# quentinll/pertrenderer

Measured on NVIDIA B200. Metric: perturbed shader fwd+bwd pixel·face·samples/sec, higher is better.
Workload: dtype f32

## Files before the change

pertrenderer_b200/csrc/cabi.cu:

```cuda
#include <math.h>

#include "kernels.h"

using namespace pert;

static thread_local const char* g_last_cuda = "none";

static int cuda_fail(int e) {
    g_last_cuda = cudaGetErrorName((cudaError_t)e);
    return PERT_E_CUDA;
}
static int cuda_rc(int e) { return e == 0 ? PERT_OK : cuda_fail(e); }

extern "C" int pert_version(void) { return PERT_ABI_VERSION; }

extern "C" uint32_t pert_shade_fused_flags(void) {
    return PERT_F_NO_SKIP | PERT_F_SKIP_DEAD_NOISE | PERT_F_PER_SAMPLE_NOISE | PERT_F_CAUCHY | PERT_F_NO_VR | PERT_F_PHILOX7;
}

extern "C" const char* pert_last_cuda_error(void) { return g_last_cuda; }

extern "C" const char* pert_strerror(int code) {
    switch (code) {
        case PERT_OK: return "ok";
// ... 120 lines not shown
static int sparse_cap(int K, int tp) {
    int cap = tp * K / 5;
    cap = (cap + 7) & ~7;
    if (cap < 32) cap = 32;
    if (cap > tp * K) cap = (tp * K + 1) & ~1;
    return cap;
}

static bool sparse_first_ok(const pert_problem* pb, const void* worklist, bool all_phases) {
    if (!worklist || !all_phases || pb->noise_rast || pb->noise_agg) return false;
    if (pb->flags & (PERT_F_NO_SKIP | PERT_F_PER_SAMPLE_NOISE | PERT_F_CAUCHY | PERT_F_NO_VR)) return false;
    return true;
}

static bool cauchy_flags_bad(uint32_t f) {
    return (f & PERT_F_CAUCHY) &&
           (f & (PERT_F_PHILOX7 | PERT_F_NO_VR | PERT_F_SKIP_DEAD_NOISE | PERT_F_UNIFORM | PERT_F_GUMBEL));
}

static bool no_vr_flags_bad(uint32_t f) {
    return (f & PERT_F_NO_VR) && (f & (PERT_F_PHILOX7 | PERT_F_SKIP_DEAD_NOISE | PERT_F_UNIFORM | PERT_F_GUMBEL));
}

extern "C" int64_t pert_num_tiles(const pert_problem* pb) {
    if (!pb || pb->K <= 0) return 0;
    const int64_t P = pb->N * pb->H * pb->W;
    const int a = dense_tp(pb->K, P), b = sparse_tp(pb->K, P);
    const int tp = a < b ? a : b;
    return (P + tp - 1) / tp;
}

extern "C" int pert_winner_bytes(int32_t K) { return (K + 1 <= 256) ? 1 : 2; }

extern "C" int64_t pert_blob_bytes(const pert_problem* pb) {
    if (!pb || pb->K <= 0) return 0;
    const int64_t P = pb->N * pb->H * pb->W;
    const int tp = sparse_tp(pb->K, P);
    return ((P + tp - 1) / tp) * (int64_t)blob_words(tp, sparse_cap(pb->K, tp)) * 4;
}

static bool aligned16(const void* p) { return ((uintptr_t)p & 15) == 0; }

static int fwd_launch_records(FwdArgs& a, FwdArgs& fb, bool sparse) {
    const int64_t P = a.pb.N * a.pb.H * a.pb.W;
    if (sparse) {
        SmemLayout t;
        const int tp2 = sparse_tp(a.pb.K, P) / 2;
        fwd_smem_layout(tp2, tp2 * a.pb.K, t);
        if ((size_t)t.bytes * (FBT / 32) > 200 * 1024) sparse = false;
    }
    a.L = make_launch(&a.pb, sparse ? sparse_tp(a.pb.K, P) : dense_tp(a.pb.K, P));
    a.L.vec_ok = a.L.vec_ok && aligned16(a.pb.pix_to_face);
    if (sparse) a.L.cap = sparse_cap(a.pb.K, a.L.tp);
    fwd_smem_layout(a.L.tp, a.L.cap, a.L.sm);
    a.L.warp_smem = a.L.sm.bytes;
    if ((size_t)a.L.warp_smem > 200 * 1024) return PERT_E_UNSUPPORTED;
    if (a.L.ntiles > 0x7fffffff) return PERT_E_UNSUPPORTED;
    if (!sparse) return 0;
    fb = a;
    fb.blob = nullptr;
    fb.L = make_launch(&a.pb, a.L.tp / 2);
    fb.L.vec_ok = fb.L.vec_ok && aligned16(a.pb.pix_to_face);
    fb.L.warp_smem_rast = fwd_smem_layout(fb.L.tp, fb.L.cap, fb.L.sm);
    fb.L.warp_smem = fb.L.sm.bytes;
    return 1;
}

extern "C" int pert_shade_fwd(const pert_problem* pb_in, float* image, uint16_t* counts, float* rsum, void* winners,
                              uint16_t* pixstate, int32_t* hist, int32_t* worklist, void* tile_blob, void* stream) {
    int rc = check_problem(pb_in);
    if (rc) return rc;
    FwdArgs a;
    a.pb = *pb_in;
    if (!(a.pb.flags & (PERT_PH_RAST | PERT_PH_AGG | PERT_PH_BLEND))) a.pb.flags |= PERT_PH_RAST | PERT_PH_AGG | PERT_PH_BLEND;
    const uint32_t f = a.pb.flags;
    if (!counts) return PERT_E_NULL;
    if ((f & PERT_PH_RAST) && !rsum) return PERT_E_NULL;
    if ((f & PERT_PH_AGG) && (!winners || !pixstate)) return PERT_E_NULL;
    if ((f & PERT_PH_BLEND) && (!image || (!a.pb.colors && !a.pb.face_colors))) return PERT_E_NULL;
    if (((f & PERT_PH_AGG) != 0) != ((f & PERT_PH_BLEND) != 0) && !hist) return PERT_E_NULL;
    if (((uintptr_t)image & 15) || ((uintptr_t)counts & 1) || ((uintptr_t)rsum & 3) || ((uintptr_t)hist & 3) ||
        ((uintptr_t)a.pb.colors & 3) || ((uintptr_t)pixstate & 1) || ((uintptr_t)winners & 3))
        return PERT_E_ALIGN;
    if ((uintptr_t)worklist & 15) return PERT_E_ALIGN;
    const uint32_t all = PERT_PH_RAST | PERT_PH_AGG | PERT_PH_BLEND;
    if ((f & PERT_F_PHILOX7) && ((f & all) != all || hist || a.pb.noise_rast || a.pb.noise_agg)) return PERT_E_UNSUPPORTED;
    if (cauchy_flags_bad(f) || no_vr_flags_bad(f)) return PERT_E_UNSUPPORTED;
    a.image = image;
    a.counts = counts;
    a.rsum = rsum;
    a.winners = winners;
    a.pixstate = pixstate;
    a.hist = hist;
    a.worklist = worklist;
    a.blob = nullptr;
    FwdArgs fb;
    rc = fwd_launch_records(a, fb, sparse_first_ok(&a.pb, worklist, (f & all) == all && !hist));
    if (rc < 0) return rc;
    const bool sparse = rc == 1;
    if ((uintptr_t)tile_blob & 15) return PERT_E_ALIGN;
    a.blob = sparse ? (int32_t*)tile_blob : nullptr;
    cudaStream_t st = (cudaStream_t)stream;
    if (!sparse) return cuda_rc(launch_shade_fwd(a, nullptr, st));
    cudaError_t e = cudaMemsetAsync(worklist, 0, 16, st);
    if (e != cudaSuccess) return cuda_fail((int)e);
    return cuda_rc(launch_shade_fwd(a, &fb, st));
}

extern "C" int pert_shade_render(const pert_problem* pb_in, float* image, uint16_t* counts_ws, int32_t* worklist,
                                 void* stream) {
    int rc = check_problem(pb_in);
    if (rc) return rc;
    FwdArgs a = {};
    a.pb = *pb_in;
    const uint32_t f = a.pb.flags;
    if (f & (PERT_PH_RAST | PERT_PH_AGG | PERT_PH_BLEND | PERT_PH_BWD_SAMPLE | PERT_PH_BWD_FINISH)) return PERT_E_UNSUPPORTED;
    if (a.pb.s_rast_begin != 0 || a.pb.s_rast_end != a.pb.S_rast || a.pb.s_agg_begin != 0 || a.pb.s_agg_end != a.pb.S_agg)
        return PERT_E_UNSUPPORTED;
    if (!image || (!a.pb.colors && !a.pb.face_colors)) return PERT_E_NULL;
    if (((uintptr_t)image & 15) || ((uintptr_t)counts_ws & 1) || ((uintptr_t)a.pb.colors & 3) || ((uintptr_t)worklist & 15))
        return PERT_E_ALIGN;
    if ((f & PERT_F_PHILOX7) && (a.pb.noise_rast || a.pb.noise_agg)) return PERT_E_UNSUPPORTED;
    if (cauchy_flags_bad(f) || no_vr_flags_bad(f)) return PERT_E_UNSUPPORTED;
    if (f & PERT_F_NO_VR) a.pb.flags |= PERT_F_PER_SAMPLE_NOISE;
    const bool sparse_ok = sparse_first_ok(&a.pb, worklist, true);
    if (sparse_ok && !counts_ws) return PERT_E_NULL;
    a.image = image;
    a.counts = counts_ws;
    a.worklist = worklist;
    FwdArgs fb;
    rc = fwd_launch_records(a, fb, sparse_ok);
    if (rc < 0) return rc;
    cudaStream_t st = (cudaStream_t)stream;
    if (rc == 0) return cuda_rc(launch_shade_render(a, nullptr, st));
// ... 32 lines not shown
        const Launch t = make_launch(&a.pb, tp2);
        SmemLayout sl;
        bwd_smem_layout(tp2, a.pb.K, t.cap, t.sc, t.nchunks, t.win_bytes, false, true, sl);
        if ((size_t)sl.bytes * (FBT / 32) > 200 * 1024) sparse = false;
    }
    const bool ptr_ok = aligned16(a.pb.pix_to_face) && aligned16(grad_dists) && aligned16(grad_zbuf) &&
                        (a.pb.face_colors || aligned16(grad_colors));
    a.L = make_launch(&a.pb, sparse ? sparse_tp(a.pb.K, a.pb.N * a.pb.H * a.pb.W) : dense_tp(a.pb.K, a.pb.N * a.pb.H * a.pb.W));
    a.L.vec_ok = a.L.vec_ok && ptr_ok;
    if (sparse) a.L.cap = sparse_cap(a.pb.K, a.L.tp);
    if (a.L.win_bytes == 2 && ((uintptr_t)winners & 1)) return PERT_E_ALIGN;
    bwd_smem_layout(a.L.tp, a.pb.K, a.L.cap, a.L.sc, a.L.nchunks, a.L.win_bytes, sparse, a.L.lean, a.L.sm);
    a.L.warp_smem = a.L.sm.bytes;
    if ((size_t)a.L.warp_smem > 200 * 1024) return PERT_E_UNSUPPORTED;
    if (a.L.ntiles > 0x7fffffff) return PERT_E_UNSUPPORTED;
    a.grad_image = grad_image;
    a.counts = counts;
    a.rsum = rsum;
    a.winners = winners;
    a.pixstate = pixstate;
    a.grad_dists = grad_dists;
    a.grad_zbuf = grad_zbuf;
    a.grad_colors = grad_colors;
    a.partials = scalar_partials;
    a.acc = acc;
    a.pixstat = pixstat;
    a.hist = hist;
    a.worklist = worklist;
    if ((uintptr_t)tile_blob & 15) return PERT_E_ALIGN;
    a.blob = sparse ? (const int32_t*)tile_blob : nullptr;
    cudaStream_t st = (cudaStream_t)stream;
    if (!sparse) return cuda_rc(launch_shade_bwd(a, nullptr, grad_scalars, st));
    BwdArgs fb = a;
    fb.blob = nullptr;
    fb.L = make_launch(&a.pb, a.L.tp / 2);
    fb.L.vec_ok = fb.L.vec_ok && ptr_ok;
    fb.L.lean = true;
    bwd_smem_layout(fb.L.tp, a.pb.K, fb.L.cap, fb.L.sc, fb.L.nchunks, fb.L.win_bytes, false, fb.L.lean, fb.L.sm);
    fb.L.warp_smem = fb.L.sm.bytes;
    cudaError_t e = cudaMemsetAsync(worklist, 0, 16, st);
    if (e != cudaSuccess) return cuda_fail((int)e);
    return cuda_rc(launch_shade_bwd(a, &fb, grad_scalars, st));
}

static int soft_launch_record(pert_problem& pb, Launch& L, bool bwd, bool ptr_ok) {
    pb.S_rast = pb.S_agg = 4;
    pb.s_rast_begin = pb.s_agg_begin = 0;
    pb.s_rast_end = pb.s_agg_end = 4;
    pb.noise_rast = pb.noise_agg = nullptr;
    pb.face_colors = nullptr;
    int rc = check_problem(&pb);
    if (rc) return rc;
    if (!pb.colors) return PERT_E_NULL;
    L = make_launch(&pb, pick_tp(pb.K));
    L.vec_ok = L.vec_ok && ptr_ok;
    soft_smem_layout(L.tp, pb.K, bwd, L.sm);
    L.warp_smem = L.sm.bytes;
    if ((size_t)L.warp_smem > 200 * 1024) return PERT_E_UNSUPPORTED;
    return PERT_OK;
}

extern "C" int pert_soft_shade_fwd(const pert_problem* pb_in, float* image, void* stream) {
    if (!pb_in || !image) return PERT_E_NULL;
    if ((uintptr_t)image & 15) return PERT_E_ALIGN;
    pert_problem pb = *pb_in;
    Launch L;
    if (int rc = soft_launch_record(pb, L, false, aligned16(pb.pix_to_face))) return rc;
// ... 171 lines not shown
```

pertrenderer_b200/csrc/common.cuh:

```cuda
#pragma once
#include <cuda_runtime.h>
#include <math_constants.h>
#include <stdint.h>

#include "../../include/pertshade.h"

namespace pert {

constexpr int NT = 128;
constexpr int NW = NT / 32;
constexpr int FNT = 32;
constexpr int FBT = 64;
constexpr unsigned FULL = 0xffffffffu;

__device__ __forceinline__ float warp_sum(float v) {
#pragma unroll
    for (int o = 16; o > 0; o >>= 1) v += __shfl_xor_sync(FULL, v, o);
    return v;
}
__device__ __forceinline__ int warp_sum_i(int v) {
#pragma unroll
    for (int o = 16; o > 0; o >>= 1) v += __shfl_xor_sync(FULL, v, o);
    return v;
}
// ... 201 lines not shown

__device__ __forceinline__ int best_lane_shift(int n, int nq, int kmax) {
    int best_k = 0, best_c = 0x7fffffff;
#pragma unroll 1
    for (int k = 0; k <= kmax; ++k) {
        const int passes = ((n << k) + 31) >> 5;
        const int per_lane = (nq + (1 << k) - 1) >> k;
        const int c = passes * (per_lane * 100 + 24 + 6 * k);
        if (c < best_c) {
            best_c = c;
            best_k = k;
        }
    }
    return best_k;
}

__device__ __forceinline__ int batch_of(int64_t pix0, int p, int64_t HW) {
    const unsigned hw = (unsigned)HW;
    const unsigned b0 = (unsigned)pix0 / hw;
    unsigned r = (unsigned)pix0 - b0 * hw + (unsigned)p;
    unsigned b = b0;
    while (r >= hw) {
        r -= hw;
        b++;
    }
    return (int)b;
}

__host__ __device__ __forceinline__ int blob_words(int tp, int cap) { return ((2 + 7 * tp + 2 * cap) + 3) & ~3; }
__host__ __device__ __forceinline__ int blob_pix_off(int tp) { return 2 + tp; }
__host__ __device__ __forceinline__ int blob_vlist_off(int tp) { return 2 + 7 * tp; }
__host__ __device__ __forceinline__ int blob_cnt_off(int tp, int cap) { return 2 + 7 * tp + cap / 2; }
__host__ __device__ __forceinline__ int blob_zeta_off(int tp, int cap) { return 2 + 7 * tp + cap; }

__device__ __forceinline__ int entry_pixel(int e, float invK) { return __float2int_rz(((float)e + 0.5f) * invK); }

}
```

pertrenderer_b200/csrc/shade_bwd.cu:

```cuda
#include <climits>
#include "kernels.h"
#include "tile.cuh"

namespace pert {

constexpr int kNab = 8;

void bwd_smem_layout(int tp, int K, int cap, int sc, int nchunks, int win_bytes, bool compact, bool lean, SmemLayout& L) {
    const size_t ns = compact ? (size_t)cap + 2 * tp : (size_t)tp * (K + 1);
    Carver cv(L);
    cv.take(cap, 2);
    cv.take(ns > (size_t)cap ? ns : (size_t)cap, 4);
    cv.take(lean && ns > (size_t)cap ? ns : (size_t)cap, 2);
    cv.take(ns, 4);
    cv.take(ns, 4);
    cv.take(nchunks > 1 ? ns : 0, 4);
    cv.take(lean ? 0 : ns, 2);
    cv.take((size_t)(tp < kNab ? tp : kNab) * sc, 4);
    cv.take(tp + 1, 4);
    cv.take(tp, 4);
    cv.take(tp, 4);
    cv.take(compact ? tp : 0, 4);
    cv.take(compact ? tp : 0, 4);
    cv.take(tp, 1);
// ... 36 lines not shown
    float* gsel = cv.take<float>();
    float* accs = zs;
    float* t2s_own = cv.take<float>();
    float* t2s = a.L.nchunks > 1 ? t2s_own : gsel;
    uint16_t* pairs_own = cv.take<uint16_t>();
    const bool lean = a.L.lean;
    uint16_t* pairs = lean ? cnt : pairs_own;
    float* cs = cv.take<float>();
    int* vstart = cv.take<int>();
    int* pa0 = cv.take<int>();
    float* pg0 = cv.take<float>();
    int* psb = cv.take<int>();
    int* pnv = cv.take<int>();
    uint8_t* apx = cv.take<uint8_t>();
    const bool early_w = a.L.nchunks == 1 && ((sa_loc * wb) & 15) == 0 && do_sample && (((uintptr_t)a.winners) & 15) == 0;
    unsigned char* wst = cv.take<unsigned char>();
    if (early_w) {
        const unsigned char* src = reinterpret_cast<const unsigned char*>(a.winners) + pix0 * sa_loc * wb;
        const int nbytes = npx * sa_loc * wb;
#pragma unroll 1
        for (int o = lane * 16; o < nbytes; o += 32 * 16) cp_async16(wst + o, src + o);
    }

    float4 Gi = make_float4(0.f, 0.f, 0.f, 0.f);
    float zn = 1.0f, zf = 100.0f;
    int pstate = K;
    if (pvalid) {
        Gi = __ldg(reinterpret_cast<const float4*>(a.grad_image) + gp);
        const int b = pb.depth_len > 1 ? batch_of(pix0, p, a.L.HW) : 0;
        zn = __ldg(pb.znear + b);
        zf = __ldg(pb.zfar + b);
        pstate = a.pixstate[gp];
    }
    const int32_t* const bl = BLOB ? a.blob + tile * (int64_t)blob_words(tp, cap) : nullptr;
    const int nv = BLOB ? __ldg(bl) : scan_valid(pb.pix_to_face + g0, E, a.L.vec_ok, vlist, cap);
    const bool overflow = COMPACT && (BLOB ? nv < 0 : nv > cap);
    if (!overflow) {
        if (do_finish) {
            zero_fill(a.grad_dists + g0, E, a.L.vec_ok);
            zero_fill(a.grad_zbuf + g0, E, a.L.vec_ok);
            if (a.grad_colors && !FACE) zero_fill(a.grad_colors + g0 * 3, E * 3, a.L.vec_ok);
        } else {
            zero_fill(a.acc + pix0 * K1, npx * K1, false);
            if (lane < npx) {
                a.pixstat[(pix0 + lane) * 2] = 0.f;
                a.pixstat[(pix0 + lane) * 2 + 1] = 0.f;
            }
        }
    }
    if (overflow) {
        if (lane == 0) a.worklist[4 + atomicAdd(a.worklist, 1)] = (int32_t)tile;
    } else if (nv > 0 || WOVR) {
        const float gal = a.L.gal;
        PixPrep pi;
        if constexpr (BLOB) {
            const float* const colors_t = pb.colors + g0 * 3;
            const float* const rsum_t = a.rsum + g0;
            for (int i = lane; i <= tp; i += 32) vstart[i] = __ldg(bl + 1 + i);
            uint32_t* const vl32 = reinterpret_cast<uint32_t*>(vlist);
            uint32_t* const cn32 = reinterpret_cast<uint32_t*>(cnt);
            const int nw = (nv + 1) >> 1;
#pragma unroll 1
            for (int i = lane; i < nw; i += 32) {
                const uint32_t v2 = (uint32_t)__ldg(bl + blob_vlist_off(tp) + i);
                vl32[i] = v2;
                cn32[i] = (uint32_t)__ldg(bl + blob_cnt_off(tp, cap) + i);
                const int e0 = v2 & 0xffff, e1 = v2 >> 16;
                if (!FACE) prefetch_l1(colors_t + e0 * 3);
                prefetch_l1(rsum_t + e0);
                if (2 * i + 1 < nv) {
                    if (!FACE) prefetch_l1(colors_t + e1 * 3);
                    prefetch_l1(rsum_t + e1);
                }
            }
#pragma unroll 1
            for (int i = lane; i < nv; i += 32) zs[i] = __int_as_float(__ldg(bl + blob_zeta_off(tp, cap) + i));
            if (pvalid) {
                const int32_t* const bp = bl + blob_pix_off(tp) + 6 * p;
                pi.zmax = __int_as_float(__ldg(bp));
                pi.zimax = __int_as_float(__ldg(bp + 1));
                pi.prod_nz = __int_as_float(__ldg(bp + 2));
                pi.zeta_max = __int_as_float(__ldg(bp + 3));
                const int w4 = __ldg(bp + 4), w5 = __ldg(bp + 5);
                pi.argzi = w4 & 0xffff;
                pi.a0 = w4 >> 16;
                pi.nzero = w5 & 0xffff;
                pi.kpad = w5 >> 16;
            } else {
                pi.zmax = pb.eps;
                pi.zimax = 0.f;
                pi.prod_nz = 1.f;
                pi.zeta_max = 0.f;
                pi.argzi = pi.a0 = pi.nzero = pi.kpad = 0;
            }
            pi.zbg = __fadd_rn(pb.eps, -pi.zmax);
            __syncwarp();
        } else {
            __syncwarp();
            pixel_ranges(vlist, nv, K, tp, vstart);
            {
                const float* const zbuf_t = pb.zbuf + g0;
                const uint16_t* const counts_t = a.counts + g0;
                const float* const colors_t = pb.colors + g0 * 3;
                const float* const rsum_t = a.rsum + g0;
#pragma unroll 1
                for (int n = lane; n < nv; n += 32) {
                    const int e = vlist[n];
                    zs[n] = __ldg(zbuf_t + e);
                    cnt[n] = counts_t[e];
// ... 358 lines not shown
                            float* gc = gfc + 3 * (int)__ldg(p2f_p + k);
                            atomicAdd(gc, w * Gi.x);
                            atomicAdd(gc + 1, w * Gi.y);
                            atomicAdd(gc + 2, w * Gi.z);
                        } else {
                            float* gc = gc_t + e * 3;
                            gc[0] = w * Gi.x;
                            gc[1] = w * Gi.y;
                            gc[2] = w * Gi.z;
                        }
                    }
                }
            }
        }
    }

    if (do_finish) {
        p_sigma = warp_sum(p_sigma);
        p_gamma = warp_sum(p_gamma);
        p_q = warp_sum(p_q);
        if (lane == 0) reinterpret_cast<float4*>(a.partials)[prow] = make_float4(p_sigma, p_gamma, p_q, 0.f);
    }
}

constexpr int BWD_MAIN_CTAS = 28;
template <class NoiseA, int GT, bool PHASED, bool FACE, bool COMPACT, bool BLOB, int SCORE = 0, bool WOVR = false>
__global__ void __launch_bounds__(FNT, BWD_MAIN_CTAS) shade_bwd_kernel(const BwdArgs a, const NoiseA noise_a) {
    extern __shared__ __align__(16) unsigned char smem_raw[];
    NoiseA na = noise_a;
    if (a.pb.seed_device) na.mix(__ldg(a.pb.seed_device + 1));
    shade_bwd_tile<NoiseA, GT, PHASED, FACE, COMPACT, BLOB, SCORE, WOVR>(a, na, blockIdx.x, blockIdx.x, smem_raw, threadIdx.x);
}

template <class NoiseA, int GT, bool FACE>
__global__ void __launch_bounds__(FBT, 12) shade_bwd_fallback_kernel(const BwdArgs a, const NoiseA noise_a, int64_t prow0) {
    extern __shared__ __align__(16) unsigned char smem_all[];
    unsigned char* smem_raw = smem_all + (threadIdx.x >> 5) * a.L.warp_smem;
    const int n = 2 * a.worklist[0];
    NoiseA na = noise_a;
    if (a.pb.seed_device) na.mix(__ldg(a.pb.seed_device + 1));
#pragma unroll 1
    for (;;) {
        int i = 0;
        if ((threadIdx.x & 31) == 0) i = n > 0 ? atomicAdd(a.worklist + 1, 1) : 0;
        i = __shfl_sync(FULL, i, 0);
        if (i >= n) break;
        const int64_t tile = (int64_t)a.worklist[4 + (i >> 1)] * 2 + (i & 1);
        if (tile < a.L.ntiles) {
            shade_bwd_tile<NoiseA, GT, false, FACE, false, false>(a, na, tile, prow0 + i, smem_raw, threadIdx.x & 31);
        } else if ((threadIdx.x & 31) == 0) {
            reinterpret_cast<float4*>(a.partials)[prow0 + i] = make_float4(0.f, 0.f, 0.f, 0.f);
        }
        __syncwarp();
    }
}

__global__ void __launch_bounds__(1024) finalize_scalars_kernel(const float* partials, int64_t n, const int32_t* worklist,
                                                                float gamma, float alpha, float* out) {
    __shared__ double red[3][32];
    if (worklist) n += 2 * (int64_t)worklist[0];
    double s0 = 0, s1 = 0, s2 = 0;
    const float4* const rows = reinterpret_cast<const float4*>(partials);
    int64_t t = threadIdx.x;
    for (; t + 7 * 1024 < n; t += 8 * 1024) {
        float4 v[8];
#pragma unroll
        for (int u = 0; u < 8; ++u) v[u] = __ldg(rows + t + u * 1024);
#pragma unroll
        for (int u = 0; u < 8; ++u) {
            s0 += v[u].x;
            s1 += v[u].y;
            s2 += v[u].z;
        }
    }
    for (; t < n; t += 1024) {
        const float4 v = __ldg(rows + t);
        s0 += v.x;
        s1 += v.y;
        s2 += v.z;
    }
#pragma unroll
    for (int o = 16; o > 0; o >>= 1) {
// ... 19 lines not shown
        out[2] = (float)(-q * (double)gamma / ((double)alpha * (double)alpha));
    }
}

template <class K>
static int set_smem(K kern, size_t smem) {
    if (smem > 48 * 1024) return (int)cudaFuncSetAttribute(kern, cudaFuncAttributeMaxDynamicSharedMemorySize, (int)smem);
    return 0;
}

template <class NA, int GT, bool PHASED, bool FACE, bool COMPACT, bool BLOB = false, int SCORE = 0, bool WOVR = false>
static int launch_bwd_f(const BwdArgs& a, const NA& na, cudaStream_t st) {
    const size_t smem = (size_t)a.L.warp_smem;
    if (int rc = set_smem(shade_bwd_kernel<NA, GT, PHASED, FACE, COMPACT, BLOB, SCORE, WOVR>, smem)) return rc;
    shade_bwd_kernel<NA, GT, PHASED, FACE, COMPACT, BLOB, SCORE, WOVR><<<(unsigned)a.L.ntiles, FNT, smem, st>>>(a, na);
    return (int)cudaGetLastError();
}
template <class NA, int GT, bool PHASED, int SCORE = 0, bool WOVR = false>
static int launch_bwd_t(const BwdArgs& a, const NA& na, cudaStream_t st) {
    return a.pb.face_colors ? launch_bwd_f<NA, GT, PHASED, true, false, false, SCORE, WOVR>(a, na, st)
                            : launch_bwd_f<NA, GT, PHASED, false, false, false, SCORE, WOVR>(a, na, st);
}
template <class PN, int GT>
static int launch_bwd_c(const BwdArgs& a, const PN& na, cudaStream_t st) {
    if (a.blob) {
        if constexpr (GT == 2 || GT == 4) {
            return a.pb.face_colors ? launch_bwd_f<PN, GT, false, true, true, true>(a, na, st)
                                    : launch_bwd_f<PN, GT, false, false, true, true>(a, na, st);
        }
    }
    return a.pb.face_colors ? launch_bwd_f<PN, GT, false, true, true>(a, na, st)
                            : launch_bwd_f<PN, GT, false, false, true>(a, na, st);
}
template <class PN, int GT, bool FACE>
static int launch_bwd_fb(const BwdArgs& a, const PN& na, int64_t prow0, cudaStream_t st) {
    const size_t smem = (size_t)a.L.warp_smem * (FBT / 32);
    if (int rc = set_smem(shade_bwd_fallback_kernel<PN, GT, FACE>, smem)) return rc;
    shade_bwd_fallback_kernel<PN, GT, FACE><<<resident_grid(shade_bwd_fallback_kernel<PN, GT, FACE>, FBT, smem), FBT, smem, st>>>(a, na, prow0);
    return (int)cudaGetLastError();
}

template <class PN>
static int launch_bwd_production(const BwdArgs& a, const BwdArgs* fb, cudaStream_t st) {
    const PN pa(a.pb.seed_agg, 1, a.pb.pixel_offset);
    int rc;
    if (fb) {
        switch (a.L.G) {
            case 1: rc = launch_bwd_c<PN, 1>(a, pa, st); break;
            case 2: rc = launch_bwd_c<PN, 2>(a, pa, st); break;
            case 4: rc = launch_bwd_c<PN, 4>(a, pa, st); break;
            default: rc = launch_bwd_c<PN, 8>(a, pa, st); break;
        }
        if (rc) return rc;
        const bool face = a.pb.face_colors != nullptr;
        switch (fb->L.G) {
            case 2: return face ? launch_bwd_fb<PN, 2, true>(*fb, pa, a.L.ntiles, st) : launch_bwd_fb<PN, 2, false>(*fb, pa, a.L.ntiles, st);
            case 4: return face ? launch_bwd_fb<PN, 4, true>(*fb, pa, a.L.ntiles, st) : launch_bwd_fb<PN, 4, false>(*fb, pa, a.L.ntiles, st);
            case 8: return face ? launch_bwd_fb<PN, 8, true>(*fb, pa, a.L.ntiles, st) : launch_bwd_fb<PN, 8, false>(*fb, pa, a.L.ntiles, st);
            default: return face ? launch_bwd_fb<PN, 16, true>(*fb, pa, a.L.ntiles, st) : launch_bwd_fb<PN, 16, false>(*fb, pa, a.L.ntiles, st);
        }
    }
    switch (a.L.G) {
        case 1: return launch_bwd_t<PN, 1, false>(a, pa, st);
        case 2: return launch_bwd_t<PN, 2, false>(a, pa, st);
        case 4: return launch_bwd_t<PN, 4, false>(a, pa, st);
        default: return launch_bwd_t<PN, 8, false>(a, pa, st);
    }
}

int launch_shade_bwd(const BwdArgs& a, const BwdArgs* fb, float* grad_scalars, cudaStream_t st) {
    int rc;
    const uint32_t both = PERT_PH_BWD_SAMPLE | PERT_PH_BWD_FINISH;
// ... 40 lines not shown
```

pertrenderer_b200/csrc/shade_fwd.cu:

```cuda
#include "kernels.h"
#include "tile.cuh"

namespace pert {

int fwd_smem_layout(int tp, int cap, SmemLayout& L) {
    Carver cv(L);
    cv.take(cap, 2);
    cv.take(cap + tp, 4);
    cv.take(cap, 2);
    cv.take(cap + tp, 4);
    cv.take(cap + tp, 2);
    cv.take(64, 2);
    const int rast_bytes = L.bytes;
    cv.take(cap, 4);
    cv.take(tp + 1, 4);
    cv.take(tp, 4);
    cv.take(tp, 2);
    return rast_bytes;
}

constexpr int kDeferMin = 48;
constexpr int kCmpMin = 12;

template <class NoiseR, class NoiseA, int GT, bool PHASED, bool DEFER = false, int CPH = 0x70, int SCORE = 0,
          bool WOVR = false, bool RENDER = false>
__device__ __forceinline__ void shade_fwd_tile(const FwdArgs& a, const NoiseR& noise_r, const NoiseA& noise_a,
                                               const int64_t tile, unsigned char* smem_raw, const int lane) {
    const pert_problem& pb = a.pb;
    const int G = GT ? GT : a.L.G;
    const int gshift = GT ? (GT == 16 ? 4 : GT == 8 ? 3 : GT == 4 ? 2 : GT == 2 ? 1 : 0) : a.L.gshift;
    const int K = pb.K, K1 = K + 1, tp = 32 >> gshift;
    const int64_t pix0 = tile * tp;
    const int npx = (int)min((int64_t)tp, a.L.P - pix0);
    const int E = npx * K;
    const int64_t g0 = pix0 * K;
    const uint32_t flags = pb.flags;
    const bool do_rast = PHASED ? (flags & PERT_PH_RAST) != 0 : (CPH & PERT_PH_RAST) != 0,
               do_agg = PHASED ? (flags & PERT_PH_AGG) != 0 : (CPH & PERT_PH_AGG) != 0,
               do_blend = PHASED ? (flags & PERT_PH_BLEND) != 0 : (CPH & PERT_PH_BLEND) != 0;
    int32_t* const ghist = PHASED ? a.hist : nullptr;
    const float* const zbuf_t = pb.zbuf + g0;
    const float* const dists_t = pb.dists + g0;
    uint16_t* const counts_t = a.counts + g0;
    float* const rsum_t = a.rsum + g0;
    const bool no_skip = flags & PERT_F_NO_SKIP;
    const int p = lane >> gshift, lig = lane & (G - 1);
    const bool pvalid = p < npx;
    const int64_t gp = pix0 + p;
    const unsigned lt = (1u << lane) - 1u;

    Taker cv(smem_raw, a.L.sm);
    uint16_t* vlist = cv.take<uint16_t>();
    float* xs = cv.take<float>();
    uint16_t* cnt = cv.take<uint16_t>();
    float* rs = cv.take<float>();
    uint16_t* rlist = cv.take<uint16_t>();
    uint16_t* ring = cv.take<uint16_t>();
    float* zs = cv.take<float>();
    int* vstart = cv.take<int>();
    int* pinfo = cv.take<int>();
    uint16_t* plist = cv.take<uint16_t>();
    const int cap = a.L.cap;
    float* lz = xs;
    int* hl = reinterpret_cast<int*>(rs);
    uint16_t* lj = rlist;

    const int nv = scan_valid(pb.pix_to_face + g0, E, a.L.vec_ok, vlist, cap);
    const int sa_loc = a.L.sa_loc;
    if (nv > cap) {
        if (lane == 0) {
            a.worklist[4 + atomicAdd(a.worklist, 1)] = (int32_t)tile;
            if (a.blob) a.blob[tile * (int64_t)blob_words(tp, cap)] = -1;
        }
        return;
    }
    if (nv == 0) {
        if (do_agg && ghist) {
#pragma unroll 1
            for (int i = lane; i < npx * K1; i += 32) ghist[pix0 * K1 + i] = ((i % K1) == K) ? sa_loc : 0;
        }
        if (!RENDER && do_agg && lane < npx) a.pixstate[pix0 + lane] = (uint16_t)K;
        if (!PHASED && !RENDER && a.blob && lane == 0) a.blob[tile * (int64_t)blob_words(tp, a.L.cap)] = 0;
        if (do_blend && lane < npx)
            reinterpret_cast<float4*>(a.image)[pix0 + lane] =
                make_float4(pb.background[0], pb.background[1], pb.background[2], 0.0f);
        return;
    }
    __syncwarp();
    if (do_agg || do_blend) pixel_ranges(vlist, nv, K, tp, vstart);

    const int sr_loc = pb.s_rast_end - pb.s_rast_begin;
    const float thr = (NoiseR::kBounded && !no_skip) ? pb.sigma * kNoiseAbsMax * 1.0001f : CUDART_INF_F;
    const bool compound = !WOVR && NoiseR::kBounded && !no_skip && !(flags & PERT_F_PER_SAMPLE_NOISE);
    const float x_cmp = compound ? a.L.t_compound * pb.sigma : CUDART_INF_F;
    uint16_t* const blist = rlist + cap - 1;
    int nlist = 0, nblist = 0;
#pragma unroll 1
    for (int n0 = 0; n0 < nv; n0 += 32) {
        const int n = n0 + lane;
        bool need = false, cmp = false;
        if (n < nv) {
            const int e = vlist[n];
            if (do_agg || do_blend) {
                zs[n] = __ldg(zbuf_t + e);
                if (!pb.face_colors) prefetch_l1(pb.colors + (g0 + e) * 3);
            }
            if (do_rast) {
                const float x = -__ldg(dists_t + e);
                xs[n] = x;
                need = WOVR ? x >= -thr : fabsf(x) <= thr;
                cmp = need && fabsf(x) >= x_cmp;
                if (!need) {
                    cnt[n] = (x >= 0.0f) ? (uint16_t)sr_loc : (uint16_t)0;
                    if constexpr (!RENDER) rs[n] = 0.0f;
                }
            } else {
                cnt[n] = counts_t[e];
            }
        }
        if (do_rast) {
            if constexpr (DEFER) {
                const unsigned b = __ballot_sync(FULL, need);
                if (need) rlist[nlist + __popc(b & lt)] = (uint16_t)n;
                nlist += __popc(b);
                nblist += __popc(__ballot_sync(FULL, cmp));
            } else {
                const unsigned b = __ballot_sync(FULL, need && !cmp), bc = __ballot_sync(FULL, cmp);
                if (need && !cmp) rlist[nlist + __popc(b & lt)] = (uint16_t)n;
                if (cmp) blist[-(nblist + __popc(bc & lt))] = (uint16_t)n;
                nlist += __popc(b);
                nblist += __popc(bc);
            }
        }
    }
    __syncwarp();
    if (do_rast) {
        if constexpr (DEFER) {
            if (nblist >= kDeferMin) {
                if (lane == 0) {
                    a.worklist[4 + atomicAdd(a.worklist, 1)] = (int32_t)tile;
                    if (a.blob) a.blob[tile * (int64_t)blob_words(tp, cap)] = -1;
                }
                return;
            }
        }
        if (!DEFER && nblist > 0 && nblist < kCmpMin) {
            const int moved = lane < nblist ? blist[-lane] : 0;
            __syncwarp();
            if (lane < nblist) rlist[nlist + lane] = (uint16_t)moved;
            nlist += nblist;
            nblist = 0;
            __syncwarp();
        }
        if constexpr (NoiseR::kBounded && !DEFER && !WOVR) {
            if (nblist > 0) {
                const CompoundCtx<NoiseR> cc{noise_r, vlist, xs, cnt, rs, K, a.L.invK, pix0, a.L.inv_sigma, sr_loc,
                                             0x40000000u + 2u * (uint32_t)(pb.s_rast_begin >> 2)};
                if constexpr (RENDER)
                    rast_compound_count_list(cc, blist, nblist, a.L.t_bucket[0] * pb.sigma, a.L.t_bucket[1] * pb.sigma, ring);
                else
                    rast_compound_list(cc, blist, nblist, a.L.t_bucket[0] * pb.sigma, a.L.t_bucket[1] * pb.sigma, ring);
            }
        }
        rast_sample_list<NoiseR, SCORE, WOVR, RENDER>(noise_r, rlist, nlist, vlist, xs, cnt, rs, K, a.L.invK, pix0, pb.sigma, a.L.inv_sigma, pb.s_rast_begin,
                         pb.s_rast_end, !no_skip, a.L.lpe_r);
        __syncwarp();
        if (!RENDER || !do_agg) {
#pragma unroll 1
            for (int n = lane; n < nv; n += 32) {
                const int e = vlist[n];
                counts_t[e] = cnt[n];
                if constexpr (!RENDER) rsum_t[e] = rs[n];
            }
        }
// ... 100 lines not shown
                        }
                    }
                    int wj[4];
#pragma unroll
                    for (int t = 0; t < 4; ++t) {
                        wj[t] = lj[plb + bi[t]];
                        const int s = q * 4 + t;
                        if (s >= pb.s_agg_begin && s < pb.s_agg_end && bi[t] != pa0) atomicAdd(&hl[plb + bi[t]], 1);
                    }
                    if constexpr (RENDER) continue;
                    const int s0 = q * 4 - pb.s_agg_begin;
                    if (pack && q * 4 + 3 < pb.s_agg_end) {
                        reinterpret_cast<uint32_t*>(a.winners)[(pgp * sa_loc + s0) >> 2] =
                            (uint32_t)wj[0] | ((uint32_t)wj[1] << 8) | ((uint32_t)wj[2] << 16) | ((uint32_t)wj[3] << 24);
                    } else {
#pragma unroll
                        for (int t = 0; t < 4; ++t)
                            if (q * 4 + t < pb.s_agg_end) store_winner(a.winners, a.L.win_bytes, pgp * sa_loc + s0 + t, wj[t]);
                    }
                }
            }
        }
        __syncwarp();
        int others = 0;
#pragma unroll 1
        for (int l = lig; l < nlive; l += G)
            if (l != a0l) others += hl[lb + l];
        others = group_sum_i(others, G);
        active = others > 0;
        if (pvalid && lig == 0) {
            hl[lb + a0l] = sa_loc - others;
            if constexpr (!RENDER) a.pixstate[gp] = (uint16_t)(pi.a0 | (active ? 0x8000 : 0));
        }
        if (!PHASED && !RENDER && a.blob) {
            int32_t* const bl = a.blob + tile * (int64_t)blob_words(tp, cap);
            if (lane == 0) bl[0] = nv;
            for (int i = lane; i <= tp; i += 32) bl[1 + i] = i <= npx ? vstart[i] : nv;
            if (pvalid && lig == 0) {
                int32_t* const bp = bl + blob_pix_off(tp) + 6 * p;
                bp[0] = __float_as_int(pi.zmax);
                bp[1] = __float_as_int(pi.zimax);
                bp[2] = __float_as_int(pi.prod_nz);
                bp[3] = __float_as_int(pi.zeta_max);
                bp[4] = pi.argzi | (pi.a0 << 16);
                bp[5] = pi.nzero | (pi.kpad << 16);
            }
            const uint32_t* const vl32 = reinterpret_cast<const uint32_t*>(vlist);
            const uint32_t* const cn32 = reinterpret_cast<const uint32_t*>(cnt);
            const int nw = (nv + 1) >> 1;
#pragma unroll 1
            for (int i = lane; i < nw; i += 32) {
                bl[blob_vlist_off(tp) + i] = (int32_t)vl32[i];
                bl[blob_cnt_off(tp, cap) + i] = (int32_t)cn32[i];
            }
#pragma unroll 1
            for (int i = lane; i < nv; i += 32) bl[blob_zeta_off(tp, cap) + i] = __float_as_int(zs[i]);
        }
        __syncwarp();
        if (ghist) {
#pragma unroll 1
            for (int i = lane; i < npx * K1; i += 32) ghist[pix0 * K1 + i] = 0;
            __syncwarp();
#pragma unroll 1
            for (int l = lig; l < nlive; l += G) ghist[gp * K1 + lj[lb + l]] = hl[lb + l];
        }
    }
    if (!do_blend) return;

    float r = 0.f, g = 0.f, bl = 0.f;
    const float fS = (float)pb.S_agg;
    const float* const colors_p = pb.colors + gp * K * 3;
    const float* const fcol = pb.face_colors;
    const int64_t* const p2f_p = pb.pix_to_face + gp * K;
    if (do_agg) {
#pragma unroll 1
        for (int l = lig; l < nlive; l += G) {
            const int hcount = hl[lb + l];
            if (hcount > 0) {
                const float w = (float)hcount / fS;
                const int j = lj[lb + l];
                if (j < K) {
                    const float* c = fcol ? fcol + 3 * (int)__ldg(p2f_p + j) : colors_p + j * 3;
                    r += w * __ldg(c);
                    g += w * __ldg(c + 1);
                    bl += w * __ldg(c + 2);
                } else {
                    r += w * pb.background[0];
                    g += w * pb.background[1];
                    bl += w * pb.background[2];
// ... 13 lines not shown
                    r += w * __ldg(c);
                    g += w * __ldg(c + 1);
                    bl += w * __ldg(c + 2);
                } else {
                    r += w * pb.background[0];
                    g += w * pb.background[1];
                    bl += w * pb.background[2];
                }
            }
        }
    }
    r = group_sum(r, G);
    g = group_sum(g, G);
    bl = group_sum(bl, G);
    if (pvalid && lig == 0) reinterpret_cast<float4*>(a.image)[gp] = make_float4(r, g, bl, px_alpha);
}

constexpr int fwd_min_ctas(int score, bool wovr, bool render) { return (score || wovr) ? 24 : render ? 28 : 32; }

template <class NoiseR, class NoiseA, int GT, bool PHASED, bool DEFER, int SCORE, bool WOVR, bool RENDER>
__global__ void __launch_bounds__(FNT, fwd_min_ctas(SCORE, WOVR, RENDER))
    shade_fwd_kernel(const FwdArgs a, const NoiseR noise_r, const NoiseA noise_a) {
    extern __shared__ __align__(16) unsigned char smem_raw[];
    NoiseR nr = noise_r;
    NoiseA na = noise_a;
    if (a.pb.seed_device) {
        nr.mix(__ldg(a.pb.seed_device));
        na.mix(__ldg(a.pb.seed_device + 1));
    }
    shade_fwd_tile<NoiseR, NoiseA, GT, PHASED, DEFER, 0x70, SCORE, WOVR, RENDER>(a, nr, na, blockIdx.x, smem_raw, threadIdx.x);
}

constexpr int FB_MIN_CTAS = 12;
template <class PN, int GT, int CPH, bool RENDER>
__global__ void __launch_bounds__(FBT, FB_MIN_CTAS) shade_fwd_fallback_kernel(const FwdArgs a, const PN noise_r, const PN noise_a) {
    extern __shared__ __align__(16) unsigned char smem_all[];
    unsigned char* smem_raw = smem_all + (threadIdx.x >> 5) * (CPH == (int)PERT_PH_RAST ? a.L.warp_smem_rast : a.L.warp_smem);
    const int n = 2 * a.worklist[0];
    PN nr = noise_r;
    PN na = noise_a;
    if (a.pb.seed_device) {
        nr.mix(__ldg(a.pb.seed_device));
        na.mix(__ldg(a.pb.seed_device + 1));
    }
#pragma unroll 1
    for (;;) {
        int i = 0;
        if ((threadIdx.x & 31) == 0) i = n > 0 ? atomicAdd(a.worklist + ((CPH & PERT_PH_RAST) ? 1 : 2), 1) : 0;
        i = __shfl_sync(FULL, i, 0);
        if (i >= n) break;
        const int64_t tile = (int64_t)a.worklist[4 + (i >> 1)] * 2 + (i & 1);
        if (tile < a.L.ntiles)
            shade_fwd_tile<PN, PN, GT, false, false, CPH, 0, false, RENDER>(a, nr, na, tile, smem_raw, threadIdx.x & 31);
        __syncwarp();
    }
}

template <class NR, class NA, int GT, bool PHASED, bool DEFER, int SCORE, bool WOVR, bool RENDER>
static int launch_t(const FwdArgs& a, const NR& nr, const NA& na, cudaStream_t st) {
    const size_t smem = (size_t)a.L.warp_smem;
    if (smem > 48 * 1024) {
        cudaError_t e = cudaFuncSetAttribute(shade_fwd_kernel<NR, NA, GT, PHASED, DEFER, SCORE, WOVR, RENDER>,
                                             cudaFuncAttributeMaxDynamicSharedMemorySize, (int)smem);
        if (e != cudaSuccess) return (int)e;
    }
    shade_fwd_kernel<NR, NA, GT, PHASED, DEFER, SCORE, WOVR, RENDER><<<(unsigned)a.L.ntiles, FNT, smem, st>>>(a, nr, na);
    return (int)cudaGetLastError();
}

template <class PN, int GT, int CPH, bool RENDER>
static int launch_fallback_ph(const FwdArgs& a, const PN& nr, const PN& na, cudaStream_t st) {
    const size_t smem = (size_t)(CPH == (int)PERT_PH_RAST ? a.L.warp_smem_rast : a.L.warp_smem) * (FBT / 32);
    if (smem > 48 * 1024) {
        cudaError_t e = cudaFuncSetAttribute(shade_fwd_fallback_kernel<PN, GT, CPH, RENDER>,
                                             cudaFuncAttributeMaxDynamicSharedMemorySize, (int)smem);
        if (e != cudaSuccess) return (int)e;
    }
    shade_fwd_fallback_kernel<PN, GT, CPH, RENDER>
        <<<resident_grid(shade_fwd_fallback_kernel<PN, GT, CPH, RENDER>, FBT, smem), FBT, smem, st>>>(a, nr, na);
    return (int)cudaGetLastError();
}

template <class PN, int GT, bool RENDER>
static int launch_fallback(const FwdArgs& a, const PN& nr, const PN& na, cudaStream_t st) {
    const int rc = launch_fallback_ph<PN, GT, PERT_PH_RAST, RENDER>(a, nr, na, st);
    return rc ? rc : launch_fallback_ph<PN, GT, PERT_PH_AGG | PERT_PH_BLEND, RENDER>(a, nr, na, st);
}

template <class PN, bool DEFER, bool RENDER>
static int launch_main(const FwdArgs& a, const PN& pr, const PN& pa, cudaStream_t st) {
    switch (a.L.G) {
        case 1: return launch_t<PN, PN, 1, false, DEFER, 0, false, RENDER>(a, pr, pa, st);
        case 2: return launch_t<PN, PN, 2, false, DEFER, 0, false, RENDER>(a, pr, pa, st);
        case 4: return launch_t<PN, PN, 4, false, DEFER, 0, false, RENDER>(a, pr, pa, st);
        default: return launch_t<PN, PN, 8, false, DEFER, 0, false, RENDER>(a, pr, pa, st);
    }
}

template <class PN, bool RENDER>
static int launch_production(const FwdArgs& a, const FwdArgs* fb, cudaStream_t st) {
    const PN pr(a.pb.seed_rast, 0, a.pb.pixel_offset), pa(a.pb.seed_agg, 1, a.pb.pixel_offset);
    if (!fb) return launch_main<PN, false, RENDER>(a, pr, pa, st);
    const int rc = launch_main<PN, true, RENDER>(a, pr, pa, st);
    if (rc) return rc;
    switch (fb->L.G) {
        case 2: return launch_fallback<PN, 2, RENDER>(*fb, pr, pa, st);
        case 4: return launch_fallback<PN, 4, RENDER>(*fb, pr, pa, st);
        case 8: return launch_fallback<PN, 8, RENDER>(*fb, pr, pa, st);
        default: return launch_fallback<PN, 16, RENDER>(*fb, pr, pa, st);
    }
}

template <class PN, int SCORE, bool WOVR, bool RENDER>
static int launch_pair(const FwdArgs& a, const FwdArgs* fb, cudaStream_t st) {
    constexpr bool PHASED = !RENDER;
    const bool er = a.pb.noise_rast != nullptr, ea = a.pb.noise_agg != nullptr;
    PN pr(a.pb.seed_rast, 0, a.pb.pixel_offset), pa(a.pb.seed_agg, 1, a.pb.pixel_offset);
    ExplicitNoise xr{a.pb.noise_rast, a.L.P, a.pb.K, a.pb.S_rast}, xa{a.pb.noise_agg, a.L.P, a.pb.K + 1, a.pb.S_agg};
    if (er && ea) return launch_t<ExplicitNoise, ExplicitNoise, 0, PHASED, false, SCORE, WOVR, RENDER>(a, xr, xa, st);
// ... 33 lines not shown
```

Before: 996.4 billion.

## Cache fallback-tile valid lists and zetas in blob for reuse across phases

Extends the tile blob with a per-half-tile record region for fallback tiles. The fallback rasterization phase writes the valid list there. The agg/blend phase and the backward fallback kernel then read it instead of rescanning pix_to_face, and backward also reads zeta values from it. This removes repeated scans of pix_to_face on overflowed or deferred tiles, at the cost of a larger blob and extra global writes.

New measurement: 1038 billion (median of 6 runs). 4.1% higher.

```diff
diff --git a/pertrenderer_b200/csrc/cabi.cu b/pertrenderer_b200/csrc/cabi.cu
--- a/pertrenderer_b200/csrc/cabi.cu
+++ b/pertrenderer_b200/csrc/cabi.cu
@@ -176,11 +176,17 @@
 
 extern "C" int pert_winner_bytes(int32_t K) { return (K + 1 <= 256) ? 1 : 2; }
 
+static int64_t blob_records_off(int K, int64_t P) {
+    const int tp = sparse_tp(K, P);
+    return ((P + tp - 1) / tp) * (int64_t)blob_words(tp, sparse_cap(K, tp));
+}
+
 extern "C" int64_t pert_blob_bytes(const pert_problem* pb) {
     if (!pb || pb->K <= 0) return 0;
     const int64_t P = pb->N * pb->H * pb->W;
     const int tp = sparse_tp(pb->K, P);
-    return ((P + tp - 1) / tp) * (int64_t)blob_words(tp, sparse_cap(pb->K, tp)) * 4;
+    const int64_t records = 2 * ((P + tp - 1) / tp) * (int64_t)fbrec_words(tp / 2, tp / 2 * pb->K);
+    return (blob_records_off(pb->K, P) + records) * 4;
 }
 
 static bool aligned16(const void* p) { return ((uintptr_t)p & 15) == 0; }
@@ -202,7 +208,7 @@
     if (a.L.ntiles > 0x7fffffff) return PERT_E_UNSUPPORTED;
     if (!sparse) return 0;
     fb = a;
-    fb.blob = nullptr;
+    fb.blob = a.blob ? a.blob + blob_records_off(a.pb.K, P) : nullptr;
     fb.L = make_launch(&a.pb, a.L.tp / 2);
     fb.L.vec_ok = fb.L.vec_ok && aligned16(a.pb.pix_to_face);
     fb.L.warp_smem_rast = fwd_smem_layout(fb.L.tp, fb.L.cap, fb.L.sm);
@@ -237,13 +243,13 @@
     a.pixstate = pixstate;
     a.hist = hist;
     a.worklist = worklist;
-    a.blob = nullptr;
+    a.blob = (int32_t*)tile_blob;
     FwdArgs fb;
     rc = fwd_launch_records(a, fb, sparse_first_ok(&a.pb, worklist, (f & all) == all && !hist));
     if (rc < 0) return rc;
     const bool sparse = rc == 1;
     if ((uintptr_t)tile_blob & 15) return PERT_E_ALIGN;
-    a.blob = sparse ? (int32_t*)tile_blob : nullptr;
+    if (!sparse) a.blob = nullptr;
     cudaStream_t st = (cudaStream_t)stream;
     if (!sparse) return cuda_rc(launch_shade_fwd(a, nullptr, st));
     cudaError_t e = cudaMemsetAsync(worklist, 0, 16, st);
@@ -342,7 +348,7 @@
     cudaStream_t st = (cudaStream_t)stream;
     if (!sparse) return cuda_rc(launch_shade_bwd(a, nullptr, grad_scalars, st));
     BwdArgs fb = a;
-    fb.blob = nullptr;
+    fb.blob = a.blob ? a.blob + blob_records_off(a.pb.K, a.L.P) : nullptr;
     fb.L = make_launch(&a.pb, a.L.tp / 2);
     fb.L.vec_ok = fb.L.vec_ok && ptr_ok;
     fb.L.lean = true;
diff --git a/pertrenderer_b200/csrc/common.cuh b/pertrenderer_b200/csrc/common.cuh
--- a/pertrenderer_b200/csrc/common.cuh
+++ b/pertrenderer_b200/csrc/common.cuh
@@ -257,6 +257,8 @@
 __host__ __device__ __forceinline__ int blob_vlist_off(int tp) { return 2 + 7 * tp; }
 __host__ __device__ __forceinline__ int blob_cnt_off(int tp, int cap) { return 2 + 7 * tp + cap / 2; }
 __host__ __device__ __forceinline__ int blob_zeta_off(int tp, int cap) { return 2 + 7 * tp + cap; }
+__host__ __device__ __forceinline__ int fbrec_words(int tp, int cap) { return ((2 + 7 * tp + cap / 2 + cap) + 3) & ~3; }
+__host__ __device__ __forceinline__ int fbrec_zeta_off(int tp, int cap) { return 2 + 7 * tp + cap / 2; }
 
 __device__ __forceinline__ int entry_pixel(int e, float invK) { return __float2int_rz(((float)e + 0.5f) * invK); }
 
diff --git a/pertrenderer_b200/csrc/shade_bwd.cu b/pertrenderer_b200/csrc/shade_bwd.cu
--- a/pertrenderer_b200/csrc/shade_bwd.cu
+++ b/pertrenderer_b200/csrc/shade_bwd.cu
@@ -92,7 +92,7 @@
         zf = __ldg(pb.zfar + b);
         pstate = a.pixstate[gp];
     }
-    const int32_t* const bl = BLOB ? a.blob + tile * (int64_t)blob_words(tp, cap) : nullptr;
+    const int32_t* const bl = BLOB ? a.blob + tile * (int64_t)(COMPACT ? blob_words(tp, cap) : fbrec_words(tp, cap)) : nullptr;
     const int nv = BLOB ? __ldg(bl) : scan_valid(pb.pix_to_face + g0, E, a.L.vec_ok, vlist, cap);
     const bool overflow = COMPACT && (BLOB ? nv < 0 : nv > cap);
     if (!overflow) {
@@ -124,7 +124,7 @@
             for (int i = lane; i < nw; i += 32) {
                 const uint32_t v2 = (uint32_t)__ldg(bl + blob_vlist_off(tp) + i);
                 vl32[i] = v2;
-                cn32[i] = (uint32_t)__ldg(bl + blob_cnt_off(tp, cap) + i);
+                if constexpr (COMPACT) cn32[i] = (uint32_t)__ldg(bl + blob_cnt_off(tp, cap) + i);
                 const int e0 = v2 & 0xffff, e1 = v2 >> 16;
                 if (!FACE) prefetch_l1(colors_t + e0 * 3);
                 prefetch_l1(rsum_t + e0);
@@ -133,8 +133,9 @@
                     prefetch_l1(rsum_t + e1);
                 }
             }
-#pragma unroll 1
-            for (int i = lane; i < nv; i += 32) zs[i] = __int_as_float(__ldg(bl + blob_zeta_off(tp, cap) + i));
+            const int zoff = COMPACT ? blob_zeta_off(tp, cap) : fbrec_zeta_off(tp, cap);
+#pragma unroll 1
+            for (int i = lane; i < nv; i += 32) zs[i] = __int_as_float(__ldg(bl + zoff + i));
             if (pvalid) {
                 const int32_t* const bp = bl + blob_pix_off(tp) + 6 * p;
                 pi.zmax = __int_as_float(__ldg(bp));
@@ -559,7 +560,7 @@
     shade_bwd_tile<NoiseA, GT, PHASED, FACE, COMPACT, BLOB, SCORE, WOVR>(a, na, blockIdx.x, blockIdx.x, smem_raw, threadIdx.x);
 }
 
-template <class NoiseA, int GT, bool FACE>
+template <class NoiseA, int GT, bool FACE, bool BLOB>
 __global__ void __launch_bounds__(FBT, 12) shade_bwd_fallback_kernel(const BwdArgs a, const NoiseA noise_a, int64_t prow0) {
     extern __shared__ __align__(16) unsigned char smem_all[];
     unsigned char* smem_raw = smem_all + (threadIdx.x >> 5) * a.L.warp_smem;
@@ -574,7 +575,7 @@
         if (i >= n) break;
         const int64_t tile = (int64_t)a.worklist[4 + (i >> 1)] * 2 + (i & 1);
         if (tile < a.L.ntiles) {
-            shade_bwd_tile<NoiseA, GT, false, FACE, false, false>(a, na, tile, prow0 + i, smem_raw, threadIdx.x & 31);
+            shade_bwd_tile<NoiseA, GT, false, FACE, false, BLOB>(a, na, tile, prow0 + i, smem_raw, threadIdx.x & 31);
         } else if ((threadIdx.x & 31) == 0) {
             reinterpret_cast<float4*>(a.partials)[prow0 + i] = make_float4(0.f, 0.f, 0.f, 0.f);
         }
@@ -660,12 +661,17 @@
     return a.pb.face_colors ? launch_bwd_f<PN, GT, false, true, true>(a, na, st)
                             : launch_bwd_f<PN, GT, false, false, true>(a, na, st);
 }
+template <class PN, int GT, bool FACE, bool BLOB>
+static int launch_bwd_fb_b(const BwdArgs& a, const PN& na, int64_t prow0, cudaStream_t st) {
+    const size_t smem = (size_t)a.L.warp_smem * (FBT / 32);
+    if (int rc = set_smem(shade_bwd_fallback_kernel<PN, GT, FACE, BLOB>, smem)) return rc;
+    shade_bwd_fallback_kernel<PN, GT, FACE, BLOB>
+        <<<resident_grid(shade_bwd_fallback_kernel<PN, GT, FACE, BLOB>, FBT, smem), FBT, smem, st>>>(a, na, prow0);
+    return (int)cudaGetLastError();
+}
 template <class PN, int GT, bool FACE>
 static int launch_bwd_fb(const BwdArgs& a, const PN& na, int64_t prow0, cudaStream_t st) {
-    const size_t smem = (size_t)a.L.warp_smem * (FBT / 32);
-    if (int rc = set_smem(shade_bwd_fallback_kernel<PN, GT, FACE>, smem)) return rc;
-    shade_bwd_fallback_kernel<PN, GT, FACE><<<resident_grid(shade_bwd_fallback_kernel<PN, GT, FACE>, FBT, smem), FBT, smem, st>>>(a, na, prow0);
-    return (int)cudaGetLastError();
+    return a.blob ? launch_bwd_fb_b<PN, GT, FACE, true>(a, na, prow0, st) : launch_bwd_fb_b<PN, GT, FACE, false>(a, na, prow0, st);
 }
 
 template <class PN>
diff --git a/pertrenderer_b200/csrc/shade_fwd.cu b/pertrenderer_b200/csrc/shade_fwd.cu
--- a/pertrenderer_b200/csrc/shade_fwd.cu
+++ b/pertrenderer_b200/csrc/shade_fwd.cu
@@ -23,7 +23,7 @@
 constexpr int kCmpMin = 12;
 
 template <class NoiseR, class NoiseA, int GT, bool PHASED, bool DEFER = false, int CPH = 0x70, int SCORE = 0,
-          bool WOVR = false, bool RENDER = false>
+          bool WOVR = false, bool RENDER = false, bool REC = false>
 __device__ __forceinline__ void shade_fwd_tile(const FwdArgs& a, const NoiseR& noise_r, const NoiseA& noise_a,
                                                const int64_t tile, unsigned char* smem_raw, const int lane) {
     const pert_problem& pb = a.pb;
@@ -64,13 +64,23 @@
     float* lz = xs;
     int* hl = reinterpret_cast<int*>(rs);
     uint16_t* lj = rlist;
-
-    const int nv = scan_valid(pb.pix_to_face + g0, E, a.L.vec_ok, vlist, cap);
+    auto blob_of = [&]() { return a.blob + tile * (int64_t)(CPH == 0x70 ? blob_words(tp, cap) : fbrec_words(tp, cap)); };
+
+    int nv;
+    if constexpr (REC) {
+        const int32_t* const bl = blob_of();
+        nv = __ldg(bl);
+        const int32_t* const src = bl + blob_vlist_off(tp);
+#pragma unroll 1
+        for (int i = lane; i < ((nv + 1) >> 1); i += 32) reinterpret_cast<int32_t*>(vlist)[i] = __ldg(src + i);
+    } else {
+        nv = scan_valid(pb.pix_to_face + g0, E, a.L.vec_ok, vlist, cap);
+    }
     const int sa_loc = a.L.sa_loc;
     if (nv > cap) {
         if (lane == 0) {
             a.worklist[4 + atomicAdd(a.worklist, 1)] = (int32_t)tile;
-            if (a.blob) a.blob[tile * (int64_t)blob_words(tp, cap)] = -1;
+            if (a.blob) blob_of()[0] = -1;
         }
         return;
     }
@@ -80,13 +90,22 @@
             for (int i = lane; i < npx * K1; i += 32) ghist[pix0 * K1 + i] = ((i % K1) == K) ? sa_loc : 0;
         }
         if (!RENDER && do_agg && lane < npx) a.pixstate[pix0 + lane] = (uint16_t)K;
-        if (!PHASED && !RENDER && a.blob && lane == 0) a.blob[tile * (int64_t)blob_words(tp, a.L.cap)] = 0;
+        if (!PHASED && !RENDER && !REC && a.blob && lane == 0) blob_of()[0] = 0;
         if (do_blend && lane < npx)
             reinterpret_cast<float4*>(a.image)[pix0 + lane] =
                 make_float4(pb.background[0], pb.background[1], pb.background[2], 0.0f);
         return;
     }
     __syncwarp();
+    if constexpr (CPH == (int)PERT_PH_RAST && !RENDER) {
+        if (a.blob) {
+            int32_t* const bl = blob_of();
+            if (lane == 0) bl[0] = nv;
+#pragma unroll 1
+            for (int i = lane; i < ((nv + 1) >> 1); i += 32)
+                bl[blob_vlist_off(tp) + i] = reinterpret_cast<const int32_t*>(vlist)[i];
+        }
+    }
     if (do_agg || do_blend) pixel_ranges(vlist, nv, K, tp, vstart);
 
     const int sr_loc = pb.s_rast_end - pb.s_rast_begin;
@@ -139,7 +158,7 @@
             if (nblist >= kDeferMin) {
                 if (lane == 0) {
                     a.worklist[4 + atomicAdd(a.worklist, 1)] = (int32_t)tile;
-                    if (a.blob) a.blob[tile * (int64_t)blob_words(tp, cap)] = -1;
+                    if (a.blob) blob_of()[0] = -1;
                 }
                 return;
             }
@@ -306,9 +325,9 @@
             hl[lb + a0l] = sa_loc - others;
             if constexpr (!RENDER) a.pixstate[gp] = (uint16_t)(pi.a0 | (active ? 0x8000 : 0));
         }
-        if (!PHASED && !RENDER && a.blob) {
-            int32_t* const bl = a.blob + tile * (int64_t)blob_words(tp, cap);
-            if (lane == 0) bl[0] = nv;
+        if (!PHASED && !RENDER && (CPH == 0x70 || REC) && a.blob) {
+            int32_t* const bl = blob_of();
+            if (CPH == 0x70 && lane == 0) bl[0] = nv;
             for (int i = lane; i <= tp; i += 32) bl[1 + i] = i <= npx ? vstart[i] : nv;
             if (pvalid && lig == 0) {
                 int32_t* const bp = bl + blob_pix_off(tp) + 6 * p;
@@ -319,16 +338,19 @@
                 bp[4] = pi.argzi | (pi.a0 << 16);
                 bp[5] = pi.nzero | (pi.kpad << 16);
             }
-            const uint32_t* const vl32 = reinterpret_cast<const uint32_t*>(vlist);
-            const uint32_t* const cn32 = reinterpret_cast<const uint32_t*>(cnt);
-            const int nw = (nv + 1) >> 1;
-#pragma unroll 1
-            for (int i = lane; i < nw; i += 32) {
-                bl[blob_vlist_off(tp) + i] = (int32_t)vl32[i];
-                bl[blob_cnt_off(tp, cap) + i] = (int32_t)cn32[i];
-            }
-#pragma unroll 1
-            for (int i = lane; i < nv; i += 32) bl[blob_zeta_off(tp, cap) + i] = __float_as_int(zs[i]);
+            if constexpr (CPH == 0x70) {
+                const uint32_t* const vl32 = reinterpret_cast<const uint32_t*>(vlist);
+                const uint32_t* const cn32 = reinterpret_cast<const uint32_t*>(cnt);
+                const int nw = (nv + 1) >> 1;
+#pragma unroll 1
+                for (int i = lane; i < nw; i += 32) {
+                    bl[blob_vlist_off(tp) + i] = (int32_t)vl32[i];
+                    bl[blob_cnt_off(tp, cap) + i] = (int32_t)cn32[i];
+                }
+            }
+            const int zoff = CPH == 0x70 ? blob_zeta_off(tp, cap) : fbrec_zeta_off(tp, cap);
+#pragma unroll 1
+            for (int i = lane; i < nv; i += 32) bl[zoff + i] = __float_as_int(zs[i]);
         }
         __syncwarp();
         if (ghist) {
@@ -408,7 +430,7 @@
 }
 
 constexpr int FB_MIN_CTAS = 12;
-template <class PN, int GT, int CPH, bool RENDER>
+template <class PN, int GT, int CPH, bool RENDER, bool REC>
 __global__ void __launch_bounds__(FBT, FB_MIN_CTAS) shade_fwd_fallback_kernel(const FwdArgs a, const PN noise_r, const PN noise_a) {
     extern __shared__ __align__(16) unsigned char smem_all[];
     unsigned char* smem_raw = smem_all + (threadIdx.x >> 5) * (CPH == (int)PERT_PH_RAST ? a.L.warp_smem_rast : a.L.warp_smem);
@@ -427,7 +449,7 @@
         if (i >= n) break;
         const int64_t tile = (int64_t)a.worklist[4 + (i >> 1)] * 2 + (i & 1);
         if (tile < a.L.ntiles)
-            shade_fwd_tile<PN, PN, GT, false, false, CPH, 0, false, RENDER>(a, nr, na, tile, smem_raw, threadIdx.x & 31);
+            shade_fwd_tile<PN, PN, GT, false, false, CPH, 0, false, RENDER, REC>(a, nr, na, tile, smem_raw, threadIdx.x & 31);
         __syncwarp();
     }
 }
@@ -444,23 +466,27 @@
     return (int)cudaGetLastError();
 }
 
-template <class PN, int GT, int CPH, bool RENDER>
+template <class PN, int GT, int CPH, bool RENDER, bool REC = false>
 static int launch_fallback_ph(const FwdArgs& a, const PN& nr, const PN& na, cudaStream_t st) {
     const size_t smem = (size_t)(CPH == (int)PERT_PH_RAST ? a.L.warp_smem_rast : a.L.warp_smem) * (FBT / 32);
     if (smem > 48 * 1024) {
-        cudaError_t e = cudaFuncSetAttribute(shade_fwd_fallback_kernel<PN, GT, CPH, RENDER>,
+        cudaError_t e = cudaFuncSetAttribute(shade_fwd_fallback_kernel<PN, GT, CPH, RENDER, REC>,
                                              cudaFuncAttributeMaxDynamicSharedMemorySize, (int)smem);
         if (e != cudaSuccess) return (int)e;
     }
-    shade_fwd_fallback_kernel<PN, GT, CPH, RENDER>
-        <<<resident_grid(shade_fwd_fallback_kernel<PN, GT, CPH, RENDER>, FBT, smem), FBT, smem, st>>>(a, nr, na);
+    shade_fwd_fallback_kernel<PN, GT, CPH, RENDER, REC>
+        <<<resident_grid(shade_fwd_fallback_kernel<PN, GT, CPH, RENDER, REC>, FBT, smem), FBT, smem, st>>>(a, nr, na);
     return (int)cudaGetLastError();
 }
 
 template <class PN, int GT, bool RENDER>
 static int launch_fallback(const FwdArgs& a, const PN& nr, const PN& na, cudaStream_t st) {
     const int rc = launch_fallback_ph<PN, GT, PERT_PH_RAST, RENDER>(a, nr, na, st);
-    return rc ? rc : launch_fallback_ph<PN, GT, PERT_PH_AGG | PERT_PH_BLEND, RENDER>(a, nr, na, st);
+    if (rc) return rc;
+    if constexpr (!RENDER) {
+        if (a.blob) return launch_fallback_ph<PN, GT, PERT_PH_AGG | PERT_PH_BLEND, false, true>(a, nr, na, st);
+    }
+    return launch_fallback_ph<PN, GT, PERT_PH_AGG | PERT_PH_BLEND, RENDER>(a, nr, na, st);
 }
 
 template <class PN, bool DEFER, bool RENDER>
```
